# GATB/bcalm

Hardware: AMD Instinct MI355X
Metric: distinct k-mers/s reads->unitigs k=31 (higher is better)
Workload: dtype u64; 1 GPU; BASELINE config 3: synthetic 100000000 x 150 bp reads per GPU, k=31, abundance-min 2, 1% substitutions, 30x coverage; multi_gpu=single GPU, minimizer_size=16, log2_partitions=22

## Files before the change

bcalm_amd/csrc/k_count_fast.h:

```cpp
#pragma once
#include "k_count.h"

namespace cdbg {

#ifndef CDBG_CB_WIDE
#define CDBG_CB_WIDE 8
#endif
#ifndef CDBG_CB1
#define CDBG_CB1 24
#endif
template <int W> struct CountCap { static constexpr bool ON = W == 1; };
#ifndef CDBG_CF_BATCH
#define CDBG_CF_BATCH 192
#endif
constexpr uint32_t CF_BATCH_MEMBERS = CDBG_CF_BATCH;
static_assert(CF_BATCH_MEMBERS % 64 == 0, "whole 64-lane steps (and mask words)");
template <int W> struct CountCb { static constexpr int V = W >= 3 ? CDBG_CB_WIDE : W == 1 ? CDBG_CB1 : 16; };
template <int W> struct CountList { static constexpr bool ON = W == 1; };
#ifndef CDBG_COUNT_SHARED
#define CDBG_COUNT_SHARED 1
#endif
template <int W> struct CountShared { static constexpr bool ON = W == 2 && CDBG_COUNT_SHARED; };
constexpr uint32_t COUNT_SHARED_MEMBERS = 4096;
constexpr uint32_t CF_TRAV16 = 0x8000u;
template <int W> inline uint32_t count_fast_record_limit(int k) {
    if (!CountList<W>::ON) return COUNT_FAST_MAX_RECORDS;
    return 0x7FFFu / (uint32_t)(RecFmt<W>::CAPB - k + 1) + 1u;
}
template <int W> struct CountGeom {
    static constexpr int KMIN = W == 1 ? 3 : 32 * (W - 1);
    static constexpr int NMAX = RecFmt<W>::CAPB - KMIN + 1;
    static constexpr int MASKW = CountCap<W>::ON ? (int)(CF_BATCH_MEMBERS / 64) : (CountCb<W>::V * NMAX + 63) / 64;
    static_assert(!CountCap<W>::ON || NMAX <= (int)CF_BATCH_MEMBERS, "a record must fit a batch");
};
#ifdef CDBG_HOSTSIM
constexpr uint32_t SIFT_MS_CAP = 96;
#else
constexpr uint32_t SIFT_MS_CAP = 1280;
#endif
template <int W, int TS, int NT, int FS = 0>
struct CountFastLds {
    uint64_t keys[TS * W];
    uint32_t cnt[TS];
    uint32_t fp[FS > 0 ? FS : 1]; uint32_t fpfill;
    uint16_t mslot[FS > 0 ? (NT / 64) * SIFT_MS_CAP : 2];
    uint16_t ring[FS > 0 ? (NT / 64) * 128 : 2];
    uint64_t stage[(NT / 64) * CountCb<W>::V * RecFmt<W>::RW + 2];
    uint64_t smask[(NT / 64) * CountGeom<W>::MASKW];
    uint64_t emask[(NT / 64) * CountGeom<W>::MASKW];
    uint32_t rinfo[(NT / 64) * CountCb<W>::V];
    uint32_t wsum[NT / 64];
    uint32_t fill[2], wr[2];
    uint32_t over;
    uint64_t cbase;
};

struct CountFastParams {
    CountParams c;
    uint32_t* retry_list; uint32_t* retry_count;
    uint32_t fast_max_records;
    uint32_t skip_fill_q8;
};

template <int CAPPED> struct CountRaw;
template <> struct CountRaw<1> { uint32_t f; };
template <> struct CountRaw<0> { uint64_t a, b; };
template <> struct CountRaw<3> { uint32_t f, p; };
template <> struct CountRaw<2> { uint64_t a, b; uint32_t p; };
template <int CAPPED>
CDBG_DEV CountRaw<CAPPED> count_raw_load(const CountParams& P, uint32_t item) {
    const uint32_t i = item < P.n_items ? item : P.n_items - 1u;
    CountRaw<CAPPED> r;
    uint32_t p = i + P.item_base;
    if constexpr (CAPPED & 2) { p = P.part_list[i]; r.p = p; }
    if constexpr (CAPPED & 1) r.f = P.part_fill[p];
    else if (P.part_pairs) { r.a = P.part_off[2ull * p]; r.b = P.part_off[2ull * p + 1]; }
    else { r.a = P.part_off[p]; r.b = P.part_off[p + 1]; }
    return r;
}
struct CountRange { uint64_t rec0; uint32_t n; uint32_t p; };
template <int CAPPED>
CDBG_DEV CountRange count_raw_resolve(const CountParams& P, uint32_t item, const CountRaw<CAPPED>& w) {
    CountRange r; r.p = item + P.item_base; r.rec0 = 0; r.n = 0;
    if (item >= P.n_items) return r;
    if constexpr (CAPPED & 2) r.p = uni_u32(w.p);
    if constexpr (CAPPED & 1) { const uint32_t f = uni_u32(w.f); r.rec0 = (uint64_t)r.p * P.part_stride; r.n = f > P.part_stride ? 0u : f; }
    else { const uint64_t a = uni_u64(w.a), b = uni_u64(w.b); r.rec0 = a; r.n = (uint32_t)(b - a); }
    return r;
}
template <int NW>
CDBG_DEV void count_wave_share(const CountRange& rg, int wave, uint64_t& w0, uint64_t& w1) {
    const uint64_t per_wave = ((uint64_t)rg.n + NW - 1) / NW;
    const uint64_t end = rg.rec0 + rg.n;
    w0 = rg.rec0 + (uint64_t)wave * per_wave;
    if (w0 > end) w0 = end;
    w1 = (w0 + per_wave < end) ? w0 + per_wave : end;
}
template <int W> struct CountBal { static constexpr bool ON = W > 2; };
template <int W, int NW>
CDBG_DEV void count_share(const CountRange& rg, int wave, uint64_t& w0, uint64_t& w1) {
    if (CountBal<W>::ON) { w0 = rg.rec0; w1 = rg.rec0 + rg.n; }
    else count_wave_share<NW>(rg, wave, w0, w1);
}
template <int W>
CDBG_DEV void count_load_chunk(const CountParams& P, uint64_t first, uint64_t end, int lane, RecView<W>& R) {
    constexpr int RW = RecFmt<W>::RW;
#pragma unroll
    for (int i = 0; i < RW; ++i) R.r[i] = 0;
    if (first + (uint64_t)lane < end) {
#pragma unroll
        for (int i = 0; i < RW; ++i) R.r[i] = P.records[(first + lane) * RW + i];
    }
}
struct CountAcc { uint32_t dist, sh, st, last_fill; uint64_t occ;
#ifdef CDBG_PROFILE_PHASES
    uint64_t ph[8], t_prev;
#endif
};
#if defined(CDBG_PROFILE_PHASES) && !defined(CDBG_HOSTSIM)
#define CDBG_FPH(i) do { const uint64_t t_ = clock64(); acc.ph[i] += t_ - acc.t_prev; acc.t_prev = t_; } while (0)
#else
#define CDBG_FPH(i) do { } while (0)
#endif
template <int W, int CAPPED>
struct CountSet { RecView<W> R; CountRaw<CAPPED> raw; };
template <int W, int CAPPED>
struct CountAhead { CountSet<W, CAPPED>* cur; CountSet<W, CAPPED>* nxt; CountRange rg_nxt; uint32_t item_nxt, item_nn; bool issued; };
template <int W, int NW, int CAPPED>
CDBG_DEV void count_issue_ahead(const CountParams& P, CountAhead<W, CAPPED>& A, int wave, int lane) {
    A.rg_nxt = count_raw_resolve<CAPPED>(P, A.item_nxt, A.cur->raw);
    uint64_t w0, w1; count_share<W, NW>(A.rg_nxt, wave, w0, w1);
    count_load_chunk<W>(P, w0, w1, lane, A.nxt->R);
    A.nxt->raw = count_raw_load<CAPPED>(P, A.item_nn);
    A.issued = true;
}

template <int W, int TS, int NT, int CAPPED, int FS = 0>
CDBG_DEV bool count_partition_fast(const CountParams& P, CountFastLds<W, TS, NT, FS>& L, const CountRange& rg, CountAhead<W, CAPPED>& A,
                                   const uint32_t par, uint64_t& chunk_base, uint32_t& chunk_left, CountAcc& acc) {
    constexpr bool SIFT = FS > 0;
    static_assert(!SIFT || W > 1, "the sifting tier is written for multi-word k-mers");
    constexpr int LOG_FS = FS == 16384 ? 14 : FS == 8192 ? 13 : FS == 4096 ? 12 : FS == 2048 ? 11 : 0;
    static_assert(!SIFT || LOG_FS > 0, "fingerprint table size");
    constexpr int RW = RecFmt<W>::RW;
    constexpr int NW = NT / 64;
    constexpr int MASKW = CountGeom<W>::MASKW;
    constexpr int LOG_TS = TS == 8192 ? 13 : TS == 4096 ? 12 : TS == 2048 ? 11 : TS == 1024 ? 10 : TS == 512 ? 9 : -1;
    static_assert(LOG_TS > 0, "table size");
    const int tid = threadIdx.x, lane = tid & 63, wave = (int)uni_u32((uint32_t)tid >> 6);
    const int k = P.k;
    constexpr int COUNT_CB = CountCb<W>::V;
    uint64_t* const stage = L.stage + (size_t)wave * COUNT_CB * RW;
    uint64_t* const smask = L.smask + (size_t)wave * MASKW;
    uint64_t* const emask = L.emask + (size_t)wave * MASKW;
    uint32_t* const rinfo = L.rinfo + (size_t)wave * COUNT_CB;
    const uint64_t lane_le = lane == 63 ? ~0ULL : ((2ULL << lane) - 1ULL);
    const uint32_t RBITS = 64u * RW;
    const uint64_t kmask1 = ~0ULL >> (64 - 2 * (k < 32 ? k : 31));

    uint64_t w0, w1; count_share<W, NW>(rg, wave, w0, w1);
    CDBG_FPH(0);
    uint32_t n_new = 0, n_fp = 0;
    uint32_t n_once = 0;
    constexpr uint32_t LCAP = (uint32_t)(TS / NW);
    const uint32_t lbase = (uint32_t)wave * LCAP;
    bool shared_done = false;
    if constexpr (CountShared<W>::ON && FS == 0) {
        constexpr uint32_t SREC = (uint32_t)(NW * COUNT_CB);
        static_assert(NW * MASKW >= (int)(COUNT_SHARED_MEMBERS / 64), "the pooled masks must cover COUNT_SHARED_MEMBERS positions");
        if (rg.n <= SREC) {
            const RecView<W>& R = A.cur->R;
            const uint32_t nrec_w = (uint32_t)(w1 - w0);
            const uint32_t nfull = (uint32_t)lane < nrec_w ? (uint32_t)R.n() : 0u;
            const uint32_t incl = wave_incl_sum_u32(nfull);
            const bool odd = __any((uint32_t)lane < nrec_w && nfull == 0u);
            const uint32_t wtot = wave_readlane_u32(incl, 63);
            if (lane == 0) L.wsum[wave] = odd ? COUNT_SHARED_MEMBERS + 1u : wtot;
            CDBG_LDS_BARRIER();
            uint32_t base = 0, total = 0;
#pragma unroll
            for (int w = 0; w < NW; ++w) { const uint32_t v = uni_u32(L.wsum[w]); if (w < wave) base += v; total += v; }
            if (total <= COUNT_SHARED_MEMBERS) {
                shared_done = true;
                if ((uint32_t)lane < nrec_w) {
                    const uint32_t gi = (uint32_t)(w0 - rg.rec0) + (uint32_t)lane;
#pragma unroll
                    for (int i = 0; i < RW; ++i) L.stage[gi * RW + i] = R.r[i];
                    const uint32_t excl = base + incl - nfull, meta = (uint32_t)R.r[0];
                    const uint32_t f0 = (meta >> 10) & 1u, f1 = (meta >> 11) & 1u, ft = (meta >> 8) & 1u, lt = (meta >> 9) & 1u;
                    L.rinfo[gi] = (RBITS - 2u * (uint32_t)k + 2u * excl) | (f1 << 31) | (f0 << 30) | (f0 << 29) | (f1 << 28) | (ft << 27) | (lt << 26);
                    atomic_or_u64(&L.smask[excl >> 6], 1ULL << (excl & 63u));
                    const uint32_t last = excl + nfull - 1u;
                    if (f1 | lt) atomic_or_u64(&L.emask[last >> 6], 1ULL << (last & 63u));
                }
                if (!A.issued) { CDBG_FPH(1); count_issue_ahead<W, NW, CAPPED>(P, A, wave, lane); }
                CDBG_LDS_BARRIER();
                const uint32_t words = (total + 63u) >> 6;
                const uint32_t pc = (uint32_t)lane < words ? (uint32_t)__popcll(L.smask[lane]) : 0u;
                const uint32_t before_word = wave_incl_sum_u32(pc) - pc;
                for (uint32_t g0 = 64u * (uint32_t)wave; g0 < total; g0 += 64u * (uint32_t)NW) {
                    const uint32_t wi = g0 >> 6;
                    const uint64_t M = uni_u64(L.smask[wi]), E = uni_u64(L.emask[wi]);
                    const uint32_t started = wave_readlane_u32(before_word, (int)wi);
                    const uint32_t g = g0 + (uint32_t)lane;
                    bool is_new = false;
                    if (g < total) {
                        const uint32_t slot = started + (uint32_t)__popcll(M & lane_le) - 1u;
                        const uint32_t ri = L.rinfo[slot];
                        const uint32_t sh = (ri & 0x3FFFu) - 2u * g;
                        const uint32_t as_first = lane_pick_u32(M, ri, lane), as_last = lane_pick_u32(E, ri, lane);
                        const uint32_t facts = (as_first & 0x68000000u) | (as_last & ~0x68000000u);
                        const bool trav = (facts & 0x0C000000u) != 0u;
                        const uint32_t* dw = reinterpret_cast<const uint32_t*>(L.stage + slot * RW) + (sh >> 5);
                        uint32_t in[2 * W + 1];
#pragma unroll
                        for (int j = 0; j < 2 * W + 1; ++j) in[j] = dw[j];
                        Kmer<W> fw;
#pragma unroll
                        for (int i = 0; i < W; ++i)
                            fw.w[i] = ((uint64_t)alignbit_u32(in[2 * i + 2], in[2 * i + 1], sh) << 32) | alignbit_u32(in[2 * i + 1], in[2 * i], sh);
                        fw.mask(k);
                        const Kmer<W> rc = fw.rc(k);
                        const bool rev = rc < fw;
                        const Kmer<W>& can = rev ? rc : fw;
                        const uint64_t ktop = can.w[W - 1] | ((uint64_t)((rev ? facts << 2 : facts) & 0xC0000000u) << 32);
                        uint32_t s = can.hash_lds() >> (32 - LOG_TS);
                        const uint64_t top = ktop, ptop = key_pending(ktop);
                        uint32_t probes = 0;
                        bool hit = false;
#pragma clang loop unroll(disable)
                        do {
                            uint64_t* const slotp = &L.keys[(uint64_t)s * W];
                            const uint64_t old = atomic_cas_u64(slotp + (W - 1), KEY_EMPTY, ptop);
                            bool eq = true;
                            if (W == 2) {
                                CDBG_COMPILER_BARRIER();
                                eq = slotp[0] == can.w[0];
                            } else if (old == top) {
#pragma unroll
                                for (int i = 0; i < W - 1; ++i) eq &= (slotp[i] == can.w[i]);
                            }
                            const bool mine = old == KEY_EMPTY, same = (old == top) & eq, wait = old == ptop;
                            if (wait) CDBG_SPIN_YIELD();
                            if (mine) {
#pragma unroll
                                for (int i = 0; i < W - 1; ++i) slotp[i] = can.w[i];
                                CDBG_LDS_FENCE();
                                atomic_exch_u64(slotp + (W - 1), top);
                            }
                            is_new = is_new | mine; hit = mine | same;
                            const bool advance = !(hit | wait);
                            s = advance ? ((s + 1) & (TS - 1)) : s; probes += advance ? 1u : 0u;
                        } while (!hit && probes < 64u);
                        if (!hit) L.over = 1;
                        else {
                            atomic_add_u32(&L.cnt[s], 1u);
                            if (trav) atomic_or_u32(&L.cnt[s], TRAV_FLAG);
                        }
                    }
                    n_new += (uint32_t)__popcll(__ballot(is_new));
                }
            }
        }
    }
    if (!shared_done)
#pragma clang loop unroll(disable)
    for (int phase = SIFT ? 0 : 1; phase < 2; ++phase) {
    RecView<W> R = A.cur->R;
    uint32_t mbase = 0;
    for (uint64_t c0 = w0; c0 < w1; c0 += 64) {
        if (c0 != w0) count_load_chunk<W>(P, c0, w1, lane, R);
        const int nrec = (int)((w1 - c0) < 64 ? (w1 - c0) : 64);
        const uint32_t nfull = lane < nrec ? (uint32_t)R.n() : 0u;
        uint32_t n = nfull, first = 0;
        if (CountBal<W>::ON) {
            const uint32_t gi = wave_incl_sum_u32(nfull), mc = wave_readlane_u32(gi, 63), ge = gi - nfull;
            const uint32_t m_lo = mc * (uint32_t)wave / (uint32_t)NW, m_hi = mc * ((uint32_t)wave + 1u) / (uint32_t)NW;
            const uint32_t sb = ge > m_lo ? ge : m_lo, se = gi < m_hi ? gi : m_hi;
            n = se > sb ? se - sb : 0u; first = sb - ge;
        }
        const uint32_t incl = wave_incl_sum_u32(n);
        const int fa = CountBal<W>::ON ? (int)uni_u32((uint32_t)__builtin_ctzll(__ballot(n != 0u) | (1ULL << 63))) : 0;
        for (int lo = 0, nb = COUNT_CB; lo < nrec; lo += nb) {
            const uint32_t before = lo ? wave_readlane_u32(incl, lo - 1) : 0u;
            if (CountCap<W>::ON) {
                const uint64_t fit = __ballot(lane >= lo && lane < lo + COUNT_CB && lane < nrec && incl - before <= CF_BATCH_MEMBERS);
                nb = (int)uni_u32((uint32_t)__popcll(fit));
            }
            const uint32_t total = wave_readlane_u32(incl, lo + nb - 1 < 63 ? lo + nb - 1 : 63) - before;
            const uint32_t excl = incl - n - before;
            if (CountBal<W>::ON && total == 0u && A.issued) continue;
            if (lane >= lo && lane < lo + nb && n) {
                const int si = lane - (fa > lo ? fa : lo);
#pragma unroll
                for (int i = 0; i < RW; ++i) stage[si * RW + i] = R.r[i];
                const uint32_t meta = (uint32_t)R.r[0];
                const uint32_t head = first == 0u ? meta : 0u, tail = first + n == nfull ? meta : 0u;
                const uint32_t f0 = (head >> 10) & 1u, f1 = (tail >> 11) & 1u, ft = (head >> 8) & 1u, lt = (tail >> 9) & 1u;
                rinfo[si] = (RBITS - 2u * (uint32_t)k - 2u * first + 2u * excl) | (f1 << 31) | (f0 << 30) | (f0 << 29) | (f1 << 28) | (ft << 27) | (lt << 26);
                atomic_or_u64(&smask[excl >> 6], 1ULL << (excl & 63u));
                const uint32_t last = excl + n - 1u;
                if (f1 | lt) atomic_or_u64(&emask[last >> 6], 1ULL << (last & 63u));
            }
            CDBG_WAVE_SYNC();
            if (!A.issued) { CDBG_FPH(1); count_issue_ahead<W, NW, CAPPED>(P, A, wave, lane); }
            if constexpr (SIFT) if (phase == 1) {
                static_assert(!SIFT || (COUNT_CB <= 8 && COUNT_CB * (CountGeom<W>::NMAX < 255 ? CountGeom<W>::NMAX : 255) <= 2048), "ring entry: 11 bits of member position (a record holds at most 255 members: its 8-bit field), 3 bits of record");
                uint16_t* const ring = L.ring + (size_t)wave * 128;
                const uint16_t* const ms = L.mslot + (size_t)wave * SIFT_MS_CAP;
                uint32_t rn = 0, rhead = 0;
                auto heavy = [&](const uint32_t cnt) {
                    bool is_new = false;
                    if ((uint32_t)lane < cnt) {
                        const uint32_t e = ring[(rhead + (uint32_t)lane) & 127u];
                        const uint32_t g = e & 0x7FFu, slot = (e >> 11) & 7u;
                        const uint32_t ri = rinfo[slot];
                        const uint32_t sh = (ri & 0x1FFFu) - 2u * g;
                        const uint32_t isf = (uint32_t)(smask[g >> 6] >> (g & 63u)) & 1u, isl = (uint32_t)(emask[g >> 6] >> (g & 63u)) & 1u;
                        const uint32_t facts = ((isf ? ri : 0u) & 0x68000000u) | ((isl ? ri : 0u) & ~0x68000000u);
                        const bool trav = (facts & 0x0C000000u) != 0u;
                        const uint32_t* dw = reinterpret_cast<const uint32_t*>(stage + slot * RW) + (sh >> 5);
                        uint32_t in[2 * W + 1];
#pragma unroll
                        for (int j = 0; j < 2 * W + 1; ++j) in[j] = dw[j];
                        Kmer<W> fw;
#pragma unroll
                        for (int i = 0; i < W; ++i)
                            fw.w[i] = ((uint64_t)alignbit_u32(in[2 * i + 2], in[2 * i + 1], sh) << 32) | alignbit_u32(in[2 * i + 1], in[2 * i], sh);
                        fw.mask(k);
                        const Kmer<W> rc = fw.rc(k);
                        const bool rev = rc < fw;
                        const Kmer<W>& can = rev ? rc : fw;
                        const uint64_t ktop = can.w[W - 1] | ((uint64_t)((rev ? facts << 2 : facts) & 0xC0000000u) << 32);
                        const uint32_t hh = can.hash_lds();
                        uint32_t s = hh >> (32 - LOG_TS);
                        bool go = true;
                        if (e & 0x8000u) {
                            uint32_t fs = hh >> (32 - LOG_FS), probes = 0, old;
                            const uint32_t tag = (((hh ^ (hh >> 15)) * 0x2C1B3C6Du) & ~3u) | 1u;
#pragma clang loop unroll(disable)
                            for (;;) {
                                old = L.fp[fs];
                                if ((old & ~2u) == tag || old == 0u || ++probes == 64u) break;
                                fs = (fs + 1) & (FS - 1);
                            }
                            if (!(old & 2u)) { go = false; if (!trav) ++n_once; }
                        }
                        if (go) {
                            const uint64_t top = ktop, ptop = key_pending(ktop);
                            uint32_t probes = 0;
                            bool hit = false;
#pragma clang loop unroll(disable)
                            do {
                                uint64_t* const slotp = &L.keys[(uint64_t)s * W];
                                const uint64_t old = atomic_cas_u64(slotp + (W - 1), KEY_EMPTY, ptop);
                                bool eq = true;
                                if (old == top) {
#pragma unroll
                                    for (int i = 0; i < W - 1; ++i) eq &= (slotp[i] == can.w[i]);
                                }
                                const bool mine = old == KEY_EMPTY, same = (old == top) & eq, wait = old == ptop;
                                if (wait) CDBG_SPIN_YIELD();
                                if (mine) {
#pragma unroll
                                    for (int i = 0; i < W - 1; ++i) slotp[i] = can.w[i];
                                    CDBG_LDS_FENCE();
                                    atomic_exch_u64(slotp + (W - 1), top);
                                }
                                is_new = is_new | mine; hit = mine | same;
                                const bool advance = !(hit | wait);
                                s = advance ? ((s + 1) & (TS - 1)) : s; probes += advance ? 1u : 0u;
                            } while (!hit && probes < 64u);
                            if (!hit) L.over = 1;
                            else {
                                atomic_add_u32(&L.cnt[s], 1u);
                                if (trav) atomic_or_u32(&L.cnt[s], TRAV_FLAG);
                            }
                        }
                    }
                    n_new += (uint32_t)__popcll(__ballot(is_new));
                };
                uint32_t started1 = 0;
                for (uint32_t g0 = 0; g0 < total; g0 += 64) {
                    const uint64_t M = uni_u64(smask[g0 >> 6]), E = uni_u64(emask[g0 >> 6]);
                    const uint32_t g = g0 + (uint32_t)lane;
                    const uint32_t slot = started1 + (uint32_t)__popcll(M & lane_le) - 1u;
                    started1 += (uint32_t)__popcll(M);
                    bool want = false; uint32_t entry = 0;
                    if (g < total) {
                        const uint32_t mi = mbase + g;
                        entry = g | (slot << 11);
                        if (mi < SIFT_MS_CAP) {
                            const uint32_t old = L.fp[ms[mi]];
                            want = (old & 2u) != 0u;
                            if (!want) {
                                const uint32_t ri = rinfo[slot];
                                const uint32_t as_first = lane_pick_u32(M, ri, lane), as_last = lane_pick_u32(E, ri, lane);
                                if (!(((as_first & 0x68000000u) | (as_last & ~0x68000000u)) & 0x0C000000u)) ++n_once;
                            }
                        } else { want = true; entry |= 0x8000u; }
                    }
                    const uint64_t wb = __ballot(want);
                    if (want) ring[(rhead + rn + (uint32_t)__popcll(wb & (lane_le >> 1))) & 127u] = (uint16_t)entry;
                    rn += (uint32_t)__popcll(wb);
                    CDBG_WAVE_SYNC();
                    if (rn >= 64u) { heavy(64u); rhead = (rhead + 64u) & 127u; rn -= 64u; CDBG_WAVE_SYNC(); }
                }
                if (rn) { heavy(rn); }
                mbase += total;
                CDBG_WAVE_SYNC();
                if (lane < MASKW && lane <= (int)((total + 63) >> 6)) { smask[lane] = 0; emask[lane] = 0; }
                CDBG_WAVE_SYNC();
                continue;
            }
            uint32_t started = 0;
            for (uint32_t g0 = 0; g0 < total; g0 += 64) {
                const uint64_t M = uni_u64(smask[g0 >> 6]), E = uni_u64(emask[g0 >> 6]);
                const uint32_t g = g0 + (uint32_t)lane;
                const bool active = g < total;
                uint32_t slot_new = 0;
                const uint32_t slot = started + (uint32_t)__popcll(M & lane_le) - 1u;
                started += (uint32_t)__popcll(M);
                bool is_new = false;
                if (active) {
                    const uint32_t ri = rinfo[slot];
                    const uint32_t sh = (ri & 0x1FFFu) - 2u * g;
                    const uint32_t as_first = lane_pick_u32(M, ri, lane), as_last = lane_pick_u32(E, ri, lane);
                    const uint32_t facts = (as_first & 0x68000000u) | (as_last & ~0x68000000u);
                    const bool trav = (facts & 0x0C000000u) != 0u;
                    Kmer<W> fw;
                    if (W == 1) {
                        const uint32_t* dw = reinterpret_cast<const uint32_t*>(stage + slot * RW) + (sh >> 5);
                        const uint32_t d0 = dw[0], d1 = dw[1], d2 = dw[2];
                        const uint32_t lo32 = alignbit_u32(d1, d0, sh), hi32 = alignbit_u32(d2, d1, sh);
                        fw.w[0] = (((uint64_t)hi32 << 32) | lo32) & kmask1;
                    } else {
                        const uint32_t* dw = reinterpret_cast<const uint32_t*>(stage + slot * RW) + (sh >> 5);
                        uint32_t in[2 * W + 1];
#pragma unroll
                        for (int j = 0; j < 2 * W + 1; ++j) in[j] = dw[j];
#pragma unroll
                        for (int i = 0; i < W; ++i)
                            fw.w[i] = ((uint64_t)alignbit_u32(in[2 * i + 2], in[2 * i + 1], sh) << 32) | alignbit_u32(in[2 * i + 1], in[2 * i], sh);
                        fw.mask(k);
                    }
                    const Kmer<W> rc = fw.rc(k);
                    const bool rev = rc < fw;
                    const Kmer<W>& can = rev ? rc : fw;
                    const uint64_t ktop = can.w[W - 1] | ((uint64_t)((rev ? facts << 2 : facts) & 0xC0000000u) << 32);
                    const uint32_t hh = can.hash_lds();
                    uint32_t s = hh >> (32 - LOG_TS);
                    bool hit = true, go = true;
                    if constexpr (SIFT) {
                        uint32_t fs = hh >> (32 - LOG_FS);
                        const uint32_t tag = (((hh ^ (hh >> 15)) * 0x2C1B3C6Du) & ~3u) | 1u;
                        uint32_t probes = 0;
                        {
                            go = false;
#pragma clang loop unroll(disable)
                            for (;;) {
                                const uint32_t old = atomic_cas_u32(&L.fp[fs], 0u, tag);
                                if (old == 0u) { is_new = true; break; }
                                if ((old & ~2u) == tag) { if (!(old & 2u)) atomic_or_u32(&L.fp[fs], 2u); break; }
                                fs = (fs + 1) & (FS - 1);
                                if (++probes == 64u) { hit = false; break; }
                            }
                            if (mbase + g < SIFT_MS_CAP) L.mslot[(size_t)wave * SIFT_MS_CAP + mbase + g] = (uint16_t)fs;
                        }
                    }
                    if (!go) { if (!hit) L.over = 1; }
                    else {
                    if (W == 1) {
                        uint32_t probes = 0; uint64_t old;
#pragma clang loop unroll(disable)
                        for (;;) {
                            old = atomic_cas_u64(&L.keys[s], ~0ULL, ktop);
                            if ((old == ~0ULL) | (old == ktop) | (++probes == 64u)) break;
                            s = (s + 1) & (TS - 1);
                        }
                        is_new = old == ~0ULL;
                        hit = is_new | (old == ktop);
                    } else {
                        const uint64_t top = ktop, ptop = key_pending(ktop);
                        uint32_t probes = 0;
                        hit = false;
#pragma clang loop unroll(disable)
                        do {
                            uint64_t* const slotp = &L.keys[(uint64_t)s * W];
                            const uint64_t old = atomic_cas_u64(slotp + (W - 1), KEY_EMPTY, ptop);
                            bool eq = true;
                            if (W == 2) {
                                CDBG_COMPILER_BARRIER();
                                eq = slotp[0] == can.w[0];
                            } else if (old == top) {
#pragma unroll
                                for (int i = 0; i < W - 1; ++i) eq &= (slotp[i] == can.w[i]);
                            }
                            const bool mine = old == KEY_EMPTY, same = (old == top) & eq, wait = old == ptop;
                            if (wait) CDBG_SPIN_YIELD();
                            if (mine) {
#pragma unroll
                                for (int i = 0; i < W - 1; ++i) slotp[i] = can.w[i];
                                CDBG_LDS_FENCE();
                                atomic_exch_u64(slotp + (W - 1), top);
                            }
                            is_new = is_new | mine; hit = mine | same;
                            const bool advance = !(hit | wait);
                            s = advance ? ((s + 1) & (TS - 1)) : s; probes += advance ? 1u : 0u;
                        } while (!hit && probes < 64u);
                    }
                    if (!hit) L.over = 1;
                    else {
                        atomic_add_u32(&L.cnt[s], 1u);
                        if (trav) atomic_or_u32(&L.cnt[s], CountList<W>::ON ? CF_TRAV16 : TRAV_FLAG);
                    }
                    if (CountList<W>::ON) slot_new = s;
                    }
                }
                const uint64_t nb = __ballot(is_new);
                if (SIFT && phase == 0) { n_fp += (uint32_t)__popcll(nb); continue; }
                if (CountList<W>::ON) {
                    const uint32_t pos = n_new + (uint32_t)__popcll(nb & (lane_le >> 1));
                    if (is_new && pos < LCAP) reinterpret_cast<uint16_t*>(L.cnt)[2u * (lbase + pos) + 1u] = (uint16_t)slot_new;
                }
                n_new += (uint32_t)__popcll(nb);
            }
            CDBG_WAVE_SYNC();
            if (lane < MASKW && lane <= (int)((total + 63) >> 6)) { smask[lane] = 0; emask[lane] = 0; }
            CDBG_WAVE_SYNC();
            mbase += total;
        }
    }
    if (SIFT && phase == 0) {
        if (!A.issued) count_issue_ahead<W, NW, CAPPED>(P, A, wave, lane);
        if (lane == 0 && n_fp) atomic_add_u32(&L.fpfill, n_fp);
        CDBG_LDS_BARRIER();
        if (uni_u32(L.over) || uni_u32(L.fpfill) > (uint32_t)(FS - FS / 4)) { acc.last_fill = uni_u32(L.fpfill); return false; }
    }
    }
    if (!A.issued) count_issue_ahead<W, NW, CAPPED>(P, A, wave, lane);
    if (lane == 0 && n_new) atomic_add_u32(&L.fill[par], n_new);
    if (CountList<W>::ON && n_new > LCAP && lane == 0) L.over = 1;
    CDBG_FPH(2);
    CDBG_LDS_BARRIER();
    CDBG_FPH(3);
    const uint32_t need = uni_u32(L.fill[par]);
    if (W > 1) acc.last_fill = SIFT ? uni_u32(L.fpfill) : need;
    if (uni_u32(L.over) || need > (uint32_t)(TS - TS / 4)) return false;
    if (SIFT) { acc.dist += n_once; acc.occ += n_once; }
    if (need > chunk_left) {
        if (tid == 0) L.cbase = atomic_add_u64(P.solid_cursor, (uint64_t)COUNT_CHUNK);
        CDBG_LDS_BARRIER();
        chunk_base = uni_u64(L.cbase); chunk_left = COUNT_CHUNK;
    }
    const uint64_t obase = chunk_base;
    const bool wr_ok = obase + need <= P.solid_cap;
    if (!wr_ok && tid == 0) *P.error = 1;
    if constexpr (CountList<W>::ON) {
        uint16_t* const h16 = reinterpret_cast<uint16_t*>(L.cnt);
        for (uint32_t j0 = 0; j0 < n_new; j0 += 64u) {
            const uint32_t j = j0 + (uint32_t)lane;
            const bool valid = j < n_new;
            const uint32_t sl = valid ? (uint32_t)h16[2u * (lbase + j) + 1u] : 0u;
            const uint64_t key = L.keys[sl];
            const uint32_t cv = h16[2u * sl];
            const uint32_t cn = cv & ~CF_TRAV16; const bool trav = cv & CF_TRAV16;
            if (valid && !trav) { ++acc.dist; acc.occ += cn; }
            const bool solid = valid && cn >= P.amin;
            if (solid) { if (trav) ++acc.st; else ++acc.sh; }
            const uint64_t sb = __ballot(solid);
            uint32_t wbase = 0;
            if (sb) {
                if (lane == 0) wbase = atomic_add_u32(&L.wr[par], (uint32_t)__popcll(sb));
                wbase = wave_readlane_u32(wbase, 0);
            }
            if (solid && wr_ok) {
                const uint64_t o = obase + wbase + (uint32_t)__popcll(sb & (lane_le >> 1));
                P.solid_keys[o] = key;
                P.solid_cnt[o] = cn | (trav ? TRAV_FLAG : 0u);
            }
            if (valid) { L.keys[sl] = KEY_EMPTY; h16[2u * sl] = 0; }
        }
    } else
    {
        constexpr int SPT = TS / NT;
        static_assert(TS % NT == 0, "slots per thread");
        uint64_t topw[SPT]; uint32_t cv[SPT];
#pragma unroll
        for (int j = 0; j < SPT; ++j) { const uint32_t sl = (uint32_t)tid + (uint32_t)j * NT; topw[j] = L.keys[(uint64_t)sl * W + (W - 1)]; cv[j] = L.cnt[sl]; }
        uint32_t my_solid = 0;
#pragma unroll
        for (int j = 0; j < SPT; ++j) {
            const bool used_j = topw[j] != KEY_EMPTY;
            const uint32_t cn = cv[j] & ~TRAV_FLAG; const bool trav = cv[j] & TRAV_FLAG;
            if (used_j && !trav) { ++acc.dist; acc.occ += cn; }
            if (used_j && cn >= P.amin) { ++my_solid; if (trav) ++acc.st; else ++acc.sh; }
        }
        const uint32_t incl = wave_incl_sum_u32(my_solid);
        const uint32_t wave_total = wave_readlane_u32(incl, 63);
        uint32_t wbase = 0;
        if (lane == 0 && wave_total) wbase = atomic_add_u32(&L.wr[par], wave_total);
        wbase = wave_readlane_u32(wbase, 0);
        uint64_t o = obase + wbase + (incl - my_solid);
#pragma unroll
        for (int j = 0; j < SPT; ++j) {
            const uint32_t sl = (uint32_t)tid + (uint32_t)j * NT;
            if (topw[j] == KEY_EMPTY) continue;
            if ((cv[j] & ~TRAV_FLAG) >= P.amin && wr_ok) {
#pragma unroll
                for (int i = 0; i < W - 1; ++i) P.solid_keys[o * W + i] = L.keys[(uint64_t)sl * W + i];
                P.solid_keys[o * W + (W - 1)] = topw[j];
                P.solid_cnt[o] = cv[j];
                ++o;
            }
            L.keys[(uint64_t)sl * W + (W - 1)] = KEY_EMPTY;
            L.cnt[sl] = 0;
        }
    }
    if constexpr (SIFT) {
        uint4 z; z.x = 0; z.y = 0; z.z = 0; z.w = 0;
        for (int i = tid; i < FS / 4; i += NT) reinterpret_cast<uint4*>(L.fp)[i] = z;
        if (tid == 0) L.fpfill = 0;
    }
    if (CountShared<W>::ON && FS == 0 && shared_done) {
        for (int i = tid; i < (int)(COUNT_SHARED_MEMBERS / 64) + 1 && i < NW * MASKW; i += NT) { L.smask[i] = 0; L.emask[i] = 0; }
    }
    if (tid == 0) { L.fill[par ^ 1u] = 0; L.wr[par ^ 1u] = 0; }
    CDBG_FPH(4);
    CDBG_LDS_BARRIER();
    CDBG_FPH(5);
    const uint32_t used = uni_u32(L.wr[par]);
    chunk_base += used; chunk_left -= used;
    if (tid == 0) { P.seg_off[rg.p] = obase; P.seg_n[rg.p] = used; }
    return true;
}

template <int W, int TS, int NT, int FS>
CDBG_NOINLINE CDBG_DEV_NOINL void count_fast_clear(CountFastLds<W, TS, NT, FS>& L) {
    const int tid = threadIdx.x;
    for (uint32_t i = tid; i < (uint32_t)(FS > 0 ? FS : 1); i += NT) L.fp[i] = 0;
    if (tid == 0) L.fpfill = 0;
    for (uint32_t i = tid; i < (uint32_t)TS; i += NT) { L.keys[(uint64_t)i * W + (W - 1)] = KEY_EMPTY; L.cnt[i] = 0; }
    for (uint32_t i = tid; i < (uint32_t)((NT / 64) * CountGeom<W>::MASKW); i += NT) { L.smask[i] = 0; L.emask[i] = 0; }
    if (tid == 0) { L.fill[0] = L.fill[1] = 0; L.wr[0] = L.wr[1] = 0; L.over = 0; }
}

#ifndef CDBG_CF_WAVES2
#define CDBG_CF_WAVES2 6
#endif
template <int W, int TS, int NT, int CAPPED, int FS = 0>
__global__ void __launch_bounds__(NT, lds_waves_per_simd(sizeof(CountFastLds<W, TS, NT, FS>), NT, W == 1 ? 6 : W == 2 ? CDBG_CF_WAVES2 : 3)) k_count_fast(CountFastParams FP) {
    CDBG_SHARED CountFastLds<W, TS, NT, FS> L;
    const CountParams& P = FP.c;
    constexpr int NW = NT / 64;
    const int tid = threadIdx.x, lane = tid & 63, wave = (int)uni_u32((uint32_t)tid >> 6);
    CountAcc ca; ca.dist = 0; ca.sh = 0; ca.st = 0; ca.occ = 0; ca.last_fill = 0;
#if defined(CDBG_PROFILE_PHASES) && !defined(CDBG_HOSTSIM)
    for (int i = 0; i < 8; ++i) ca.ph[i] = 0;
    ca.t_prev = clock64();
#endif
    uint64_t chunk_base = 0; uint32_t chunk_left = 0;
    count_fast_clear<W, TS, NT, FS>(L);
    CDBG_LDS_BARRIER();
    const uint32_t stride = gridDim.x;
    CountRange rg_cur = count_raw_resolve<CAPPED>(P, blockIdx.x, count_raw_load<CAPPED>(P, blockIdx.x));
    CountSet<W, CAPPED> S0, S1;
    S0.raw = count_raw_load<CAPPED>(P, blockIdx.x + stride);
    { uint64_t w0, w1; count_share<W, NW>(rg_cur, wave, w0, w1); count_load_chunk<W>(P, w0, w1, lane, S0.R); }
    uint32_t par = 0, misses = 0, deferred = 0;
    uint32_t dpu_q8 = 0;
    auto one_partition = [&](CountSet<W, CAPPED>& cur, CountSet<W, CAPPED>& nxt, const uint32_t item) {
        CountAhead<W, CAPPED> A;
        A.cur = &cur; A.nxt = &nxt; A.item_nxt = item + stride; A.item_nn = item + 2 * stride; A.issued = false;
        if (rg_cur.n) {
            bool done = false;
            bool try_fast = misses < 4;
            if (!try_fast && ++deferred >= 16u) { try_fast = true; deferred = 0; }
            uint32_t size = rg_cur.n;
            if (W > 1 && FP.skip_fill_q8) {
                if (CountBal<W>::ON && rg_cur.n <= 64u) size = wave_readlane_u32(wave_incl_sum_u32((uint32_t)cur.R.n()), 63);
                else if (CountBal<W>::ON) size = rg_cur.n * 64u;
                if ((((uint64_t)size * dpu_q8) >> 8) * 256u > (uint64_t)(FS > 0 ? FS : TS) * FP.skip_fill_q8) try_fast = false;
            }
            if (try_fast && rg_cur.n < FP.fast_max_records) {
                done = count_partition_fast<W, TS, NT, CAPPED, FS>(P, L, rg_cur, A, par, chunk_base, chunk_left, ca);
                if (W > 1 && FP.skip_fill_q8) {
                    const uint32_t sample = (uint32_t)((float)ca.last_fill * 256.0f / (float)(size ? size : 1u));
                    dpu_q8 = dpu_q8 ? (uint32_t)((int32_t)dpu_q8 + (((int32_t)sample - (int32_t)dpu_q8) >> 4)) : sample;
                }
                if (done) { par ^= 1u; misses = 0; deferred = 0; }
                else {
                    CDBG_LDS_BARRIER();
                    count_fast_clear<W, TS, NT, FS>(L);
                    par = 0; ++misses;
                    CDBG_LDS_BARRIER();
                }
            }
            if (!done && tid == 0) {
                const uint32_t i = atomic_add_u32(FP.retry_count, 1u);
                FP.retry_list[i] = rg_cur.p;
            }
        }
        if (!A.issued) count_issue_ahead<W, NW, CAPPED>(P, A, wave, lane);
        rg_cur = A.rg_nxt;
    };
    for (uint32_t item = blockIdx.x; item < P.n_items;) {
        one_partition(S0, S1, item); item += stride;
        if (item >= P.n_items) break;
        one_partition(S1, S0, item); item += stride;
    }
#if defined(CDBG_PROFILE_PHASES) && !defined(CDBG_HOSTSIM)
    if (lane == 0 && (wave == 0 || wave == NW - 1)) for (int i = 0; i < 6; ++i) atomic_add_u64(&P.stats[8 + (wave ? 8 : 0) + i], ca.ph[i]);
#endif
    {
        uint64_t d = wave_sum_u64(ca.dist), o = wave_sum_u64(ca.occ), h = wave_sum_u64(ca.sh), t = wave_sum_u64(ca.st);
        if (lane == 0) {
            if (d) atomic_add_u64(&P.stats[0], d);
            if (o) atomic_add_u64(&P.stats[1], o);
            if (h) atomic_add_u64(&P.stats[2], h);
            if (t) atomic_add_u64(&P.stats[3], t);
        }
    }
}

}
```

Measured before the change: 25.12 billion kmers/s.

## Process two adjacent k-mers per lane in the one-word count path

Adds a pair path for one-word k-mers (enabled by default) in which each lane extracts two consecutive k-mers from one 64-bit window. The second k-mer's reverse complement is derived cheaply from the first's. Each record is sized in pairs, so a 64-lane step covers up to 128 k-mers, and mask bookkeeping shrinks to one word built with DPP wave-OR reductions. The goal is to halve the staging and step overhead per k-mer, at the cost of two serial hash probes per lane and more register pressure.

```diff
diff --git a/bcalm_amd/csrc/k_count_fast.h b/bcalm_amd/csrc/k_count_fast.h
--- a/bcalm_amd/csrc/k_count_fast.h
+++ b/bcalm_amd/csrc/k_count_fast.h
@@ -27,11 +27,37 @@
     if (!CountList<W>::ON) return COUNT_FAST_MAX_RECORDS;
     return 0x7FFFu / (uint32_t)(RecFmt<W>::CAPB - k + 1) + 1u;
 }
+#ifndef CDBG_COUNT_PAIR
+#define CDBG_COUNT_PAIR 1
+#endif
+#ifndef CDBG_COUNT_PAIR_FORM
+#define CDBG_COUNT_PAIR_FORM 0
+#endif
+template <int W> struct CountPair { static constexpr bool ON = W == 1 && CDBG_COUNT_PAIR; };
+#ifdef CDBG_HOSTSIM
+CDBG_DEV uint64_t count_wave_or_u64(uint64_t v) {
+    for (int d = 32; d >= 1; d >>= 1) v |= __shfl_xor(v, d);
+    return v;
+}
+#else
+CDBG_DEV uint32_t count_wave_or_u32(uint32_t v) {
+    v |= (uint32_t)__builtin_amdgcn_update_dpp(0, (int)v, 0x111, 0xf, 0xf, false);
+    v |= (uint32_t)__builtin_amdgcn_update_dpp(0, (int)v, 0x112, 0xf, 0xf, false);
+    v |= (uint32_t)__builtin_amdgcn_update_dpp(0, (int)v, 0x114, 0xf, 0xf, false);
+    v |= (uint32_t)__builtin_amdgcn_update_dpp(0, (int)v, 0x118, 0xf, 0xf, false);
+    v |= (uint32_t)__builtin_amdgcn_update_dpp(0, (int)v, 0x142, 0xa, 0xf, false);
+    v |= (uint32_t)__builtin_amdgcn_update_dpp(0, (int)v, 0x143, 0xc, 0xf, false);
+    return (uint32_t)__builtin_amdgcn_readlane((int)v, 63);
+}
+CDBG_DEV uint64_t count_wave_or_u64(uint64_t v) { return ((uint64_t)count_wave_or_u32((uint32_t)(v >> 32)) << 32) | count_wave_or_u32((uint32_t)v); }
+#endif
+constexpr uint32_t CF_PAIR_ODD = 1u << 25;
 template <int W> struct CountGeom {
     static constexpr int KMIN = W == 1 ? 3 : 32 * (W - 1);
     static constexpr int NMAX = RecFmt<W>::CAPB - KMIN + 1;
-    static constexpr int MASKW = CountCap<W>::ON ? (int)(CF_BATCH_MEMBERS / 64) : (CountCb<W>::V * NMAX + 63) / 64;
+    static constexpr int MASKW = CountPair<W>::ON ? 1 : CountCap<W>::ON ? (int)(CF_BATCH_MEMBERS / 64) : (CountCb<W>::V * NMAX + 63) / 64;
     static_assert(!CountCap<W>::ON || NMAX <= (int)CF_BATCH_MEMBERS, "a record must fit a batch");
+    static_assert(!CountPair<W>::ON || (NMAX + 1) / 2 <= 64, "a record's pairs must fit one step");
 };
 #ifdef CDBG_HOSTSIM
 constexpr uint32_t SIFT_MS_CAP = 96;
@@ -54,6 +80,7 @@
     uint32_t over;
     uint64_t cbase;
 };
+static_assert(sizeof(CountFastLds<1, 4096, 512>) <= 53472, "the first tier of one-word k-mers: three workgroups per CU (160 KB of LDS) depend on this size");
 
 struct CountFastParams {
     CountParams c;
@@ -263,7 +290,136 @@
             }
         }
     }
-    if (!shared_done)
+    if constexpr (CountPair<W>::ON) {
+        static_assert(!CountPair<W>::ON || (W == 1 && !SIFT && MASKW == 1 && CountList<W>::ON), "the pair path is written for one-word k-mers");
+        RecView<W> R = A.cur->R;
+#ifdef CDBG_HOSTSIM
+        uint32_t batch_no = 0;
+#endif
+        for (uint64_t c0 = w0; c0 < w1; c0 += 64) {
+            if (c0 != w0) count_load_chunk<W>(P, c0, w1, lane, R);
+            const int nrec = (int)((w1 - c0) < 64 ? (w1 - c0) : 64);
+            const uint32_t n = lane < nrec ? (uint32_t)R.n() : 0u;
+            const uint32_t np = (n + 1u) >> 1;
+            const uint32_t incl = wave_incl_sum_u32(np);
+            for (int lo = 0, nb = 1; lo < nrec; lo += nb) {
+                const uint32_t before = lo ? wave_readlane_u32(incl, lo - 1) : 0u;
+                const uint64_t fit = __ballot(lane >= lo && lane < lo + COUNT_CB && lane < nrec && incl - before <= 64u);
+                nb = (int)uni_u32((uint32_t)__popcll(fit));
+                const uint32_t total = wave_readlane_u32(incl, lo + nb - 1) - before;
+                const uint32_t excl = incl - np - before;
+                const bool staged = lane >= lo && lane < lo + nb && n;
+                const uint64_t have = __ballot(staged);
+                uint64_t sbit = 0, ebit = 0;
+                if (staged) {
+                    const uint32_t si = (uint32_t)__popcll(have & (lane_le >> 1));
+#pragma unroll
+                    for (int i = 0; i < RW; ++i) stage[si * RW + i] = R.r[i];
+                    const uint32_t meta = (uint32_t)R.r[0];
+                    const uint32_t f0 = (meta >> 10) & 1u, f1 = (meta >> 11) & 1u, ft = (meta >> 8) & 1u, lt = (meta >> 9) & 1u;
+                    rinfo[si] = (RBITS - 2u * (uint32_t)k + 4u * excl) | (f1 << 31) | (f0 << 30) | (f0 << 29) | (f1 << 28) | (ft << 27) | (lt << 26) | ((n & 1u) << 25);
+                    const uint32_t last = excl + np - 1u;
+                    sbit = 1ULL << excl;
+                    if (f1 | lt | (n & 1u)) ebit = 1ULL << last;
+#ifdef CDBG_HOSTSIM
+                    if (const char* tf = getenv("CDBG_SIM_COUNT_TRACE")) if (FILE* fp = fopen(tf, "a")) {
+                        fprintf(fp, "%u %d %u %u %u %u %u %u %u %u\n", rg.p, wave, batch_no, n, np, excl, f0, f1, ft, lt);
+                        fclose(fp);
+                    }
+#endif
+                }
+#ifdef CDBG_HOSTSIM
+                ++batch_no;
+#endif
+                CDBG_WAVE_SYNC();
+                if (!A.issued) { CDBG_FPH(1); count_issue_ahead<W, NW, CAPPED>(P, A, wave, lane); }
+                const uint64_t M = count_wave_or_u64(sbit), E = count_wave_or_u64(ebit);
+                bool new_a = false, new_b = false;
+                uint32_t slot_a = 0, slot_b = 0;
+                if ((uint32_t)lane < total) {
+                    const uint32_t slot = (uint32_t)__popcll(M & lane_le) - 1u;
+                    const uint32_t ri = rinfo[slot];
+                    const uint32_t sh = (ri & 0x1FFFu) - 4u * (uint32_t)lane - 2u;
+                    const uint32_t as_first = lane_pick_u32(M, ri, lane), as_last = lane_pick_u32(E, ri, lane);
+                    const bool single = (as_last & CF_PAIR_ODD) != 0u;
+                    const uint32_t facts_a = (as_first & 0x68000000u) | ((single ? as_last : 0u) & 0x94000000u);
+                    const uint32_t facts_b = (single ? 0u : as_last) & 0x94000000u;
+                    const uint32_t* dw = reinterpret_cast<const uint32_t*>(stage + slot * RW) + (sh >> 5);
+                    const uint32_t d0 = dw[0], d1 = dw[1], d2 = dw[2];
+                    const uint64_t x = ((uint64_t)alignbit_u32(d2, d1, sh) << 32) | alignbit_u32(d1, d0, sh);
+                    Kmer<W> fa, fb, ra, rb;
+                    fa.w[0] = (x >> 2) & kmask1; fb.w[0] = x & kmask1;
+                    ra = fa.rc(k);
+                    rb.w[0] = (ra.w[0] >> 2) | ((uint64_t)(3u - ((uint32_t)x & 3u)) << (2 * k - 2));
+                    const bool rev_a = ra < fa, rev_b = rb < fb;
+                    const Kmer<W>& ca = rev_a ? ra : fa;
+                    const Kmer<W>& cb = rev_b ? rb : fb;
+                    const uint64_t kt_a = ca.w[0] | ((uint64_t)((rev_a ? facts_a << 2 : facts_a) & 0xC0000000u) << 32);
+                    uint64_t kt_b = cb.w[0] | ((uint64_t)((rev_b ? facts_b << 2 : facts_b) & 0xC0000000u) << 32);
+                    uint32_t sa = ca.hash_lds() >> (32 - LOG_TS), sb = cb.hash_lds() >> (32 - LOG_TS);
+                    bool hit_a, hit_b;
+#if CDBG_COUNT_PAIR_FORM == 0
+                    {
+                        uint32_t probes = 0; uint64_t old;
+#pragma clang loop unroll(disable)
+                        for (;;) {
+                            old = atomic_cas_u64(&L.keys[sa], ~0ULL, kt_a);
+                            if ((old == ~0ULL) | (old == kt_a) | (++probes == 64u)) break;
+                            sa = (sa + 1) & (TS - 1);
+                        }
+                        new_a = old == ~0ULL; hit_a = new_a | (old == kt_a);
+                    }
+                    hit_b = true;
+                    if (!single) {
+                        uint32_t probes = 0; uint64_t old;
+#pragma clang loop unroll(disable)
+                        for (;;) {
+                            old = atomic_cas_u64(&L.keys[sb], ~0ULL, kt_b);
+                            if ((old == ~0ULL) | (old == kt_b) | (++probes == 64u)) break;
+                            sb = (sb + 1) & (TS - 1);
+                        }
+                        new_b = old == ~0ULL; hit_b = new_b | (old == kt_b);
+                    }
+#else
+                    {
+                        if (single) { kt_b = kt_a; sb = sa; }
+                        uint32_t probes = 0, claimed = 0; uint64_t oa, ob;
+#pragma clang loop unroll(disable)
+                        for (;;) {
+                            oa = atomic_cas_u64(&L.keys[sa], ~0ULL, kt_a);
+                            ob = atomic_cas_u64(&L.keys[sb], ~0ULL, kt_b);
+                            claimed |= (oa == ~0ULL ? 1u : 0u) | (ob == ~0ULL ? 2u : 0u);
+                            const bool ha = (oa == ~0ULL) | (oa == kt_a), hb = (ob == ~0ULL) | (ob == kt_b);
+                            if ((ha & hb) | (++probes == 64u)) break;
+                            sa = ha ? sa : ((sa + 1) & (TS - 1));
+                            sb = hb ? sb : ((sb + 1) & (TS - 1));
+                        }
+                        new_a = (claimed & 1u) != 0u; hit_a = new_a | (oa == kt_a);
+                        new_b = (claimed & 2u) != 0u; hit_b = single | new_b | (ob == kt_b);
+                    }
+#endif
+                    if (!(hit_a & hit_b)) L.over = 1;
+                    if (hit_a) {
+                        atomic_add_u32(&L.cnt[sa], 1u);
+                        if (facts_a & 0x0C000000u) atomic_or_u32(&L.cnt[sa], CF_TRAV16);
+                    }
+                    if (hit_b && !single) {
+                        atomic_add_u32(&L.cnt[sb], 1u);
+                        if (facts_b & 0x0C000000u) atomic_or_u32(&L.cnt[sb], CF_TRAV16);
+                    }
+                    slot_a = sa; slot_b = sb;
+                }
+                const uint64_t ba = __ballot(new_a), bb = __ballot(new_b);
+                const uint32_t pos_a = n_new + (uint32_t)__popcll(ba & (lane_le >> 1)) + (uint32_t)__popcll(bb & (lane_le >> 1));
+                const uint32_t pos_b = pos_a + (new_a ? 1u : 0u);
+                if (new_a && pos_a < LCAP) reinterpret_cast<uint16_t*>(L.cnt)[2u * (lbase + pos_a) + 1u] = (uint16_t)slot_a;
+                if (new_b && pos_b < LCAP) reinterpret_cast<uint16_t*>(L.cnt)[2u * (lbase + pos_b) + 1u] = (uint16_t)slot_b;
+                n_new += (uint32_t)__popcll(ba) + (uint32_t)__popcll(bb);
+                CDBG_WAVE_SYNC();
+            }
+        }
+    }
+    if (!CountPair<W>::ON && !shared_done)
 #pragma clang loop unroll(disable)
     for (int phase = SIFT ? 0 : 1; phase < 2; ++phase) {
     RecView<W> R = A.cur->R;
```

New measurement: 24.27 billion kmers/s. -3.4%, worse.
